# ParBLiSS/FastANI

Measured on AMD Instinct MI355X. Metric: ANI pairs/sec, many-to-many NxN ~5 Mbp genomes, higher is better.
Workload: dtype u32

## Files before the change

fastani_amd/csrc/engine_map.hip:

```cpp
#include <atomic>
#include <thread>
#include "host/engine.hpp"
#include "kernels/l1.hpp"
#include "kernels/l2.hpp"
#include "kernels/reduce.hpp"
#include "kernels/profile.hpp"
#include "kernels/cluster.hpp"
#include "kernels/tree.hpp"
#include "kernels/nj.hpp"
#include "kernels/single.hpp"
#include "kernels/sigdist.hpp"
#include "kernels/sigstrip.hpp"
#include "kernels/signeigh.hpp"
#include "kernels/sigscreen.hpp"
#include "kernels/sigcontain.hpp"
#include "kernels/sigcluster.hpp"
#include "kernels/siggraph.hpp"

namespace anih {
using namespace ani;

void launch_l2_codes(unsigned grid, hipStream_t s, const L2FastArgs &fa);
void launch_l2_sim_a(unsigned grid, hipStream_t s, const L2FastArgs &fa, const int32_t *list, const unsigned int *listCount);
void launch_l2_sim_b(unsigned grid, hipStream_t s, const L2FastArgs &fa, const int32_t *list, const unsigned int *listCount);
// ... 186 lines not shown
    TRY(device_scan(ctx, ctx->fragCandCntClamped.as<int32_t>(), ctx->fragOrdOff.as<uint32_t>(), (uint32_t)nF, &nCand));
    if (nCand) {
      TRY(ctx->ocFrag.ensure(nCand * 4)); TRY(ctx->ocSeq.ensure(nCand * 4)); TRY(ctx->ocStart.ensure(nCand * 4)); TRY(ctx->ocEnd.ensure(nCand * 4));
      hipLaunchKernelGGL(k_l1_order, dim3(grid_for(nF)), dim3(256), 0, ctx->stream, ctx->fragCandOff.as<uint32_t>(), ctx->fragCandCntClamped.as<int32_t>(),
                         ctx->fragOrdOff.as<uint32_t>(), fragOrder, (int32_t)nF, ctx->candSeq.as<int32_t>(), ctx->candStart.as<int32_t>(),
                             ctx->candEnd.as<int32_t>(),
                         ctx->ocFrag.as<int32_t>(), ctx->ocSeq.as<int32_t>(), ctx->ocStart.as<int32_t>(), ctx->ocEnd.as<int32_t>());
      HIP_TRY(hipGetLastError());
    }
  }
  *nCandOut = (int32_t)nCand;
  ctx->counters.l1Candidates += nCand;
  if (nCand == 0) return ANI_OK;

  TRY(ctx->l2Best.ensure(nCand * 4)); TRY(ctx->l2First.ensure(nCand * 4)); TRY(ctx->l2Last.ensure(nCand * 4));
  TRY(ctx->refStart.ensure(nCand * 4)); TRY(ctx->idBits.ensure(nCand * 4));
  {
    StageTimer tm(ctx, &ctx->counters.msL2);
    TRY(zero_counters(ctx));
    L2Args a;
    a.candFrag = ctx->ocFrag.as<int32_t>(); a.candSeq = ctx->ocSeq.as<int32_t>(); a.candStart = ctx->ocStart.as<int32_t>();
    a.candEnd = ctx->ocEnd.as<int32_t>();
    a.nCand = (int32_t)nCand; a.qPool = fs.qPool; a.fragOff = fs.fragOff; a.fragS = fs.fragS;
    a.mHash = sk->mHash; a.mWpos = sk->mWpos; a.dup = DupLinks{sk->dupList, sk->nDup, sk->dupBits}; a.mWin = sk->mWin; a.posBase = sk->posBase;
    a.posSample = sk->posSample;
    a.contigFirstMin = sk->contigFirstMin;
    { int lg = 0; while ((2 << lg) <= w) lg++; a.rankShift = 21 - std::max(0, lg - 1); }
    a.L = L; a.w = w; a.k = k; a.scratch = nullptr; a.laneStride = 0;
    a.outBest = ctx->l2Best.as<int32_t>(); a.outFirst = ctx->l2First.as<int32_t>(); a.outLast = ctx->l2Last.as<int32_t>();
    a.sumEntries = cnt_ptr(ctx, CNT_ENTRIES); a.sumSteps = cnt_ptr(ctx, CNT_STEPS); a.sumQ = cnt_ptr(ctx, CNT_SUMQ);

    uint32_t *ordOff = nullptr;
    TRY(pinned_buffer(ctx, 0, nF * 4, (void **)&ordOff));
    HIP_TRY(hipMemcpyAsync(ordOff, ctx->fragOrdOff.p, nF * 4, hipMemcpyDeviceToHost, ctx->stream));
    HIP_TRY(hipStreamSynchronize(ctx->stream));

    const size_t CH = ctx->l2ChunkCandidates;
    for (int p = 0; p < 2; p++) {
      TRY(ctx->l2Ranges[p].ensure(CH * sizeof(L2Range))); TRY(ctx->l2CodeCount[p].ensure(CH * 4)); TRY(ctx->l2CodeOff[p].ensure(CH * 4));
      TRY(ctx->l2SlowFlag[p].ensure(CH * 4)); TRY(ctx->l2ClassList[p].ensure(CH * 4));
      TRY(ctx->l2Order[p].ensure(CH * 4)); TRY(ctx->l2LenHist[p].ensure((kL2LenBuckets + 4) * 4));
    }
    TRY(ctx->l2SlowList.ensure(nCand * 4));
    HIP_TRY(hipMemsetAsync(cnt_ptr(ctx, CNT_NEG), 0, 8, ctx->stream));
    struct SideJoin { ani_ctx *c; ~SideJoin() { (void)hipStreamSynchronize(c->stream2); } } sideJoin{ctx};
    HIP_TRY(hipEventRecord(ctx->evSetDone[0], ctx->stream)); HIP_TRY(hipEventRecord(ctx->evSetDone[1], ctx->stream));
    HIP_TRY(hipStreamWaitEvent(ctx->stream2, ctx->evSetDone[1], 0));
    size_t chunk = CH;
    int nChunk = 0;
    for (size_t c0 = 0; c0 < nCand;) {
      const size_t c1 = std::min<size_t>(nCand, c0 + chunk);
      const size_t n = c1 - c0;
      const int p = nChunk & 1;
      HIP_TRY(hipEventSynchronize(ctx->evSetDone[p]));
      HIP_TRY(hipStreamWaitEvent(ctx->stream, ctx->evSetDone[p], 0));
      L2FastArgs fa;
      fa.g = a; fa.c0 = (int32_t)c0; fa.c1 = (int32_t)c1;
      fa.ranges = ctx->l2Ranges[p].as<L2Range>(); fa.codeCount = ctx->l2CodeCount[p].as<int32_t>(); fa.codeOff = ctx->l2CodeOff[p].as<uint32_t>();
      fa.codes = nullptr; fa.slowFlag = ctx->l2SlowFlag[p].as<int32_t>(); fa.fragCandOff = ctx->fragOrdOff.as<uint32_t>(); fa.fragOrder = fragOrder;
      fa.nFrag = (int32_t)nF;
      const int32_t fA = (int32_t)(std::upper_bound(ordOff, ordOff + nF, (uint32_t)c0) - ordOff) - 1;
      const int32_t fB = (int32_t)(std::upper_bound(ordOff, ordOff + nF, (uint32_t)(c1 - 1)) - ordOff) - 1;
      fa.fragBase = fA;
      { const char *ev = getenv("ANI_TEST_L2_PATH"); fa.allowFast = (ev && !strcmp(ev, "general")) ? 0 : (ev && !strcmp(ev, "classB")) ? 2 : 1; }
      if (L - (w - 1) - (k - 1) + 2 > (int)kWinMask || L - (w - 1) - (k - 1) < 1) fa.allowFast = 0;
      {
        StageTimer tk(ctx, &ctx->counters.msL2Ranges, 1);
        hipLaunchKernelGGL(k_l2_ranges, dim3(grid_for(n)), dim3(kTPB), 0, ctx->stream, fa);
      }
      fa.nFragChunk = fB - fA + 1;
      uint64_t nCodes = 0;
      {
        const int rc = device_scan(ctx, fa.codeCount, ctx->l2CodeOff[p].as<uint32_t>(), (uint32_t)n, &nCodes, ctx->l2CodeLimit);
        if (rc == ANI_ERR_LIMIT && n > 1) { chunk = (n + 1) / 2; ctx->counters.l2ChunkHalvings++; continue; }
        TRY(rc);
      }
      TRY(ctx->l2Codes[p].ensure((nCodes + 64) * 2));
      fa.codes = ctx->l2Codes[p].as<uint32_t>();
      if (nCodes) {
        {
          StageTimer tk(ctx, &ctx->counters.msL2Ranges, 1);
          HIP_TRY(hipMemsetAsync(ctx->l2LenHist[p].p, 0, kL2LenBuckets * 4, ctx->stream));
          HIP_TRY(hipMemsetD32Async((hipDeviceptr_t)(ctx->l2LenHist[p].as<unsigned int>() + kL2LenBuckets), (int)n, 1, ctx->stream));
          hipLaunchKernelGGL(k_l2_len_hist, dim3(grid_for(n, kTPB, 2048)), dim3(kTPB), 0, ctx->stream, (const int32_t *)fa.codeCount, (int32_t)n,
              ctx->l2LenHist[p].as<unsigned int>());
          hipLaunchKernelGGL(k_l2_len_scan, dim3(1), dim3(kTPB), 0, ctx->stream, ctx->l2LenHist[p].as<unsigned int>());
          hipLaunchKernelGGL(k_l2_len_scatter, dim3(grid_for(n, kTPB)), dim3(kTPB), 0, ctx->stream, (const int32_t *)fa.codeCount, (int32_t)c0, (int32_t)n,
                             ctx->l2LenHist[p].as<unsigned int>(), ctx->l2Order[p].as<int32_t>());
        }
        {
          StageTimer tk(ctx, &ctx->counters.msL2Codes, 1);
          launch_l2_codes((unsigned)((fa.nFragChunk + 7) / 8 * 8), ctx->stream, fa);
        }
        const bool overlap = ctx->l2Overlap;
        hipStream_t simStream = ctx->stream;
        if (overlap) {
          HIP_TRY(hipEventRecord(ctx->evSimA[p], ctx->stream));
          HIP_TRY(hipStreamWaitEvent(ctx->stream2, ctx->evSimA[p], 0));
          simStream = ctx->stream2;
        }
        {
          StageTimer tk(ctx, &ctx->counters.msL2Kernel, 1, simStream);
          launch_l2_sim_a(grid_for(n, kL2SimTPB), simStream, fa, (const int32_t *)ctx->l2Order[p].as<int32_t>(),
              (const unsigned int *)ctx->l2LenHist[p].as<unsigned int>() + kL2LenBuckets);
        }
        ctx->counters.l2Launches++;
      }
      HIP_TRY(hipEventRecord(ctx->evSimA[p], ctx->stream));
      HIP_TRY(hipStreamWaitEvent(ctx->stream2, ctx->evSimA[p], 0));
      if (nCodes) {
        StageTimer tk(ctx, &ctx->counters.msL2SimB, 1, ctx->stream2);
        HIP_TRY(hipMemsetAsync(cnt_ptr(ctx, CNT_CLASSB), 0, 8, ctx->stream2));
        hipLaunchKernelGGL(k_l2_collect_class, dim3(grid_for(n)), dim3(256), 0, ctx->stream2, (int32_t)c0, (int32_t)n, (const int32_t *)fa.slowFlag, 4,
                           ctx->l2ClassList[p].as<int32_t>(), (unsigned int *)cnt_ptr(ctx, CNT_CLASSB));
        L2FastArgs fb = fa;
        fb.g.sumEntries = cnt_ptr(ctx, CNT_ENTRIES_B); fb.g.sumQ = cnt_ptr(ctx, CNT_SUMQ_B); fb.g.sumSteps = cnt_ptr(ctx, CNT_STEPS_B);
        launch_l2_sim_b(grid_for(n, kL2SimTPB), ctx->stream2, fb, (const int32_t *)ctx->l2ClassList[p].as<int32_t>(), (const unsigned int *)cnt_ptr(ctx,
            CNT_CLASSB));
      }
      hipLaunchKernelGGL(k_l2_collect_slow, dim3(grid_for(n)), dim3(256), 0, ctx->stream2, (int32_t)c0, (int32_t)n, (const int32_t *)fa.slowFlag,
                         ctx->l2SlowList.as<int32_t>(), (unsigned int *)cnt_ptr(ctx, CNT_NEG), cnt_ptr(ctx, CNT_REASON));
      HIP_TRY(hipEventRecord(ctx->evSetDone[p], ctx->stream2));
      HIP_TRY(hipGetLastError());
      c0 = c1; nChunk++;
    }
    HIP_TRY(hipStreamWaitEvent(ctx->stream, ctx->evSetDone[0], 0)); HIP_TRY(hipStreamWaitEvent(ctx->stream, ctx->evSetDone[1], 0));
    unsigned long long nSlow64 = 0;
    HIP_TRY(hipMemcpyAsync(&nSlow64, cnt_ptr(ctx, CNT_NEG), 8, hipMemcpyDeviceToHost, ctx->stream));
    HIP_TRY(hipStreamSynchronize(ctx->stream));
    const size_t nSlowTotal = (size_t)(uint32_t)nSlow64;
    if (nSlowTotal) {
      size_t lanes = (std::min<size_t>(nSlowTotal, (size_t)1 << 17) + kTPB - 1) / kTPB * kTPB;
      const size_t wordsPerLane = (size_t)maxS + 1;
      while (lanes > kTPB && lanes * wordsPerLane * 4 > ((size_t)2 << 30)) lanes = (lanes / 2 + kTPB - 1) / kTPB * kTPB;
      TRY(ctx->l2Scratch.ensure(lanes * wordsPerLane * 4));
      L2Args sa = a; sa.scratch = ctx->l2Scratch.as<uint32_t>(); sa.laneStride = lanes;
      StageTimer tk(ctx, &ctx->counters.msL2Slow, 1);
      for (size_t base = 0; base < nSlowTotal; base += lanes)
        hipLaunchKernelGGL(k_l2, dim3((unsigned)(lanes / kTPB)), dim3(kTPB), 0, ctx->stream, sa, (const int32_t *)ctx->l2SlowList.as<int32_t>(),
            (int32_t)nSlowTotal, (int32_t)base);
      HIP_TRY(hipGetLastError());
    }
    ctx->counters.l2SlowCandidates += nSlowTotal; ctx->counters.l2FastCandidates += nCand - nSlowTotal;
    FinishArgs fa;
    fa.nCand = (int32_t)nCand; fa.candFrag = a.candFrag; fa.candSeq = a.candSeq; fa.best = a.outBest; fa.firstPos = a.outFirst; fa.lastPos = a.outLast;
    fa.fragS = a.fragS; fa.idLUT = set->dIdLUT; fa.minShared = set->dMinShared; fa.lutMaxS = set->dLutMaxS;
    fa.refStart = ctx->refStart.as<int32_t>(); fa.idBits = ctx->idBits.as<uint32_t>();
    hipLaunchKernelGGL(k_finish_candidates, dim3(grid_for(nCand)), dim3(256), 0, ctx->stream, fa);
    HIP_TRY(hipGetLastError());
  }
  TRY(read_counters(ctx, host));
  ctx->counters.l2WindowEntries += host[CNT_ENTRIES] + host[CNT_ENTRIES_B]; ctx->counters.l2Steps += host[CNT_STEPS] + host[CNT_STEPS_B];
  ctx->counters.l2QueryHashes += host[CNT_SUMQ] + host[CNT_SUMQ_B];
  ctx->counters.l2WindowEntriesB += host[CNT_ENTRIES_B]; ctx->counters.l2QueryHashesB += host[CNT_SUMQ_B];
  ctx->counters.l2SlowLimit += host[CNT_REASON + 1]; ctx->counters.l2SlowDup += host[CNT_REASON + 2]; ctx->counters.l2SlowOverflow += host[CNT_REASON + 3];
  return ANI_OK;
}

int reduce_stage(ani_ctx *ctx, ani_sketch *set, IndexChunk *sk, const FragSet &fs, int32_t nCand, int32_t nQuery, bool compact = false)
{
  if (nQuery == 0 || sk->nGenomes == 0) return ANI_OK;
  const size_t binsPerQuery = sk->totalBins;
  const size_t nBins = binsPerQuery * (size_t)nQuery;
  TRY(ctx->bins.ensure((nBins ? nBins : 1) * 4));
  const size_t nPairsAll = (size_t)nQuery * (size_t)(compact ? sk->nGenomes : set->nGenomes);
  TRY(ctx->rows.ensure((nPairsAll ? nPairsAll : 1) * 8));
  hipError_t e1;
  {
  StageTimer tm(ctx, &ctx->counters.msReduce);
  e1 = hipMemsetAsync(ctx->bins.p, 0, (nBins ? nBins : 1) * 4, ctx->stream);
// ... 1905 lines not shown
```

fastani_amd/csrc/kernels/l2.hpp:

```cpp
#pragma once
#include <type_traits>
#include "common.hpp"
#include "index.hpp"

namespace ani {

struct L2Result {
  int32_t best;
  int32_t firstPos;
  int32_t lastPos;
  int32_t entries;
  int32_t steps;
};

struct L2State {
  uint32_t *w;
  size_t stride;
  __host__ __device__ __forceinline__ uint32_t get(int g) const { return w[(size_t)g * stride]; }
  __host__ __device__ __forceinline__ void set(int g, uint32_t v) const { w[(size_t)g * stride] = v; }
};

__host__ __device__ __forceinline__ int32_t lower_bound_wpos(const int32_t *mWpos, int32_t lo, int32_t hi, int32_t pos)
{
  while (lo < hi) {
// ... 73 lines not shown
{
  L2Result r; r.best = 0; r.firstPos = 0; r.lastPos = 0; r.steps = 0;
  const int32_t cmw = L - (w - 1) - (k - 1);
  int32_t beg = lower_bound_wpos(mWpos, cLo, cHi, rangeStart);
  int32_t end = lower_bound_wpos(mWpos, cLo, cHi, mWpos[beg] + cmw);
  const int32_t last = lower_bound_wpos(mWpos, cLo, cHi, rangeEnd + L);
  r.entries = last - beg;
  L2Sim sim; sim.init(s, st);
  for (int32_t j = beg; j < end; j++)
    if (!dup_flag(dup, (uint32_t)j) || dup_prev(dup, (uint32_t)j) < beg) sim.insert(q_rank(q, s, mHash[j]));
  int32_t pb = beg, pe = end;
  int32_t pos = mWpos[beg];
  while (end < last) {
    if (pb != beg) {
      const int32_t nx = dup_flag(dup, (uint32_t)pb) ? dup_next(dup, (uint32_t)pb) : -1;
      if (!(nx >= 0 && nx < pe)) sim.erase(q_rank(q, s, mHash[pb]));
    }
    if (pe != end) {
      if (!dup_flag(dup, (uint32_t)pe) || dup_prev(dup, (uint32_t)pe) < beg) sim.insert(q_rank(q, s, mHash[pe]));
    }
    const int32_t wb = mWpos[beg];
    if (sim.shared > r.best) { r.best = sim.shared; r.firstPos = wb; r.lastPos = wb; }
    else if (sim.shared == r.best) r.lastPos = wb;
    r.steps++;
    pb = beg; pe = end;
    const int32_t d1 = mWpos[beg + 1] - pos;
    const int32_t d2 = mWpos[end] - (pos + cmw - 1);
    const int32_t adv = d1 < d2 ? d1 : d2;
    pos += adv;
    if (adv == d1) beg++;
    if (adv == d2) end++;
  }
  return r;
}

struct L2Args {
  const int32_t *candFrag, *candSeq, *candStart, *candEnd;
  int32_t nCand;
  const uint32_t *qPool; const uint32_t *fragOff; const int32_t *fragS;
  const uint32_t *mHash; const int32_t *mWpos; DupLinks dup;
  const uint32_t *mWin;
  const int32_t *contigFirstMin;
  const uint32_t *posBase, *posSample;
  int rankShift;
  int L, w, k;
  uint32_t *scratch; size_t laneStride;
  int32_t *outBest, *outFirst, *outLast;
  unsigned long long *sumEntries, *sumSteps, *sumQ;
};

static __global__ __launch_bounds__(kTPB) void k_l2(L2Args a, const int32_t *__restrict__ list, int32_t listCount, int32_t listBase)
{
  const int32_t lane = blockIdx.x * blockDim.x + threadIdx.x;
  const int32_t li = listBase + lane;
  unsigned long long e = 0, st = 0, sq = 0;
  if (li < listCount && (size_t)lane < a.laneStride) {
    const int32_t c = list ? list[li] : li;
    const int32_t f = a.candFrag[c];
    const int32_t seq = a.candSeq[c];
    L2State state; state.w = a.scratch + lane; state.stride = a.laneStride;
    L2Result r = l2_candidate(a.qPool + a.fragOff[f], a.fragS[f], a.mHash, a.mWpos, a.dup,
                              a.contigFirstMin[seq], a.contigFirstMin[seq + 1], a.candStart[c], a.candEnd[c],
                              a.L, a.w, a.k, state);
    a.outBest[c] = r.best; a.outFirst[c] = r.firstPos; a.outLast[c] = r.lastPos;
    e = (unsigned long long)r.entries; st = (unsigned long long)r.steps; sq = (unsigned long long)a.fragS[f];
  }
#pragma unroll
  for (int d = 32; d > 0; d >>= 1) { e += __shfl_down(e, d); st += __shfl_down(st, d); sq += __shfl_down(sq, d); }
  if ((threadIdx.x & 63) == 0 && (e | st | sq)) { atomicAdd(stat_slot(a.sumEntries), e); atomicAdd(stat_slot(a.sumSteps), st);
    atomicAdd(stat_slot(a.sumQ), sq); }
}

constexpr int kL2FastMaxS = 319;
constexpr int kL2FastMaxEntries = 16384;
template <int MAXS>
struct L2Geom {
  static constexpr int kMaxS = MAXS;
  static constexpr int kStateWords = (MAXS + 1 + 3) / 4;
  static constexpr int kWords = kStateWords;
};
using L2GeomA = L2Geom<255>;
using L2GeomB = L2Geom<319>;
constexpr int kL2SimTPB = 64;

struct L2Range { int32_t beg0, end0, last, nEvents; };

struct L2FastArgs {
  L2Args g;
  int32_t c0, c1;
  L2Range *ranges;
  int32_t *codeCount;
  const uint32_t *codeOff;
  uint32_t *codes;
  int32_t *slowFlag;
  const uint32_t *fragCandOff;
  const int32_t *fragOrder;
  int32_t nFrag, fragBase, nFragChunk;
  int32_t allowFast;
};

__device__ __forceinline__ int32_t l2_search_pos(const L2Args &g, uint32_t pb, int32_t nb, int32_t cHi, int32_t pos)
{
  int32_t bin = (pos < 0 ? 0 : pos) >> kPosSampleShift; bin = bin < nb ? bin : nb - 1;
  const int32_t lo = (int32_t)g.posSample[pb + (uint32_t)bin];
  const int32_t hi = bin + 1 < nb ? (int32_t)g.posSample[pb + (uint32_t)bin + 1] : cHi;
  return lower_bound_wpos(g.mWpos, lo, hi, pos);
}

static __global__ __launch_bounds__(kTPB) void k_l2_ranges(L2FastArgs a)
{
  const int32_t c = a.c0 + blockIdx.x * blockDim.x + threadIdx.x;
  if (c >= a.c1) return;
  const int32_t i = c - a.c0;
  const int32_t seq = a.g.candSeq[c];
  const int32_t cLo = a.g.contigFirstMin[seq], cHi = a.g.contigFirstMin[seq + 1];
  const int32_t cmw = a.g.L - (a.g.w - 1) - (a.g.k - 1);
  L2Range r;
  const uint32_t pb = a.g.posBase[seq]; const int32_t nb = (int32_t)(a.g.posBase[seq + 1] - pb);
  auto search = [&](int32_t pos) -> int32_t { return l2_search_pos(a.g, pb, nb, cHi, pos); };
  r.beg0 = search(a.g.candStart[c]);
  const int32_t wposBeg0 = a.g.mWpos[r.beg0];
  r.end0 = search(wposBeg0 + cmw);
  r.last = search(a.g.candEnd[c] + a.g.L);
  const int32_t m = r.last - r.beg0;
  const int32_t s = a.g.fragS[a.g.candFrag[c]];
  const bool fast = a.allowFast && s >= 1 && s <= kL2FastMaxS && m >= 1 && m <= kL2FastMaxEntries;
  int32_t nEv = 0;
  if (fast && r.end0 < r.last) {
    const int32_t lastDel = (r.last - 1) - (int32_t)(a.g.mWin[r.last - 1] & kWinMask) - 2;
    const int32_t nDel = lastDel >= r.beg0 ? lastDel - r.beg0 + 1 : 0;
    nEv = (r.end0 - r.beg0) + (r.last - 1 - r.end0) + nDel;
  }
  r.nEvents = nEv;
  a.ranges[i] = r;
  if (fast && nEv == 0) {
    a.g.outBest[c] = 0; a.g.outFirst[c] = 0; a.g.outLast[c] = 0;
    a.codeCount[i] = 0; a.slowFlag[i] = 16;
    return;
  }
  a.codeCount[i] = fast ? ((nEv + 8) & ~7) : 0;
  a.slowFlag[i] = fast ? ((s <= L2GeomA::kMaxS && a.allowFast != 2) ? 0 : 4) : 1;
}

constexpr uint32_t kL2DupBit = 1u << 10, kL2InsBit = 1u << 11, kL2NoEvalBit = 1u << 12;
constexpr int kL2DeltaShift = 13;
static_assert((kWinDupBit >> 21) == kL2DupBit && (kWinMoreBit >> 18) == kL2NoEvalBit, "flag bits of the window links shift into the event code");
constexpr int kL2RankBuckets = 2048;
__device__ __forceinline__ int l2_rank_bucket(uint32_t h, int sh) { const uint32_t b = h >> sh;
  return (int)(b < (uint32_t)(kL2RankBuckets - 1) ? b : (uint32_t)(kL2RankBuckets - 1)); }

__device__ __forceinline__ void l2_rank_table(const uint32_t *__restrict__ q, int s, int sh, uint32_t *qs, uint32_t *st2, uint32_t *cnt2, int *scanScratch)
{
  static_assert(kL2FastMaxS <= 2 * kTPB && kL2RankBuckets == 8 * kTPB, "two sketch hashes and eight buckets per thread");
  { uint4 z; z.x = z.y = z.z = z.w = 0u; ((uint4 *)cnt2)[threadIdx.x] = z; }
  const int i0 = (int)threadIdx.x, i1 = (int)threadIdx.x + kTPB;
  const uint32_t q0 = i0 < s ? q[i0] : 0xffffffffu, q1 = i1 < s ? q[i1] : 0xffffffffu;
  if (i0 < s) qs[i0] = q0;
  if (i1 < s) qs[i1] = q1;
  if (threadIdx.x < 2) qs[s + threadIdx.x] = 0xffffffffu;
  block_barrier();
  if (i0 < s) { const int b = l2_rank_bucket(q0, sh); atomicAdd(&cnt2[b >> 1], 1u << ((b & 1) << 4)); }
  if (i1 < s) { const int b = l2_rank_bucket(q1, sh); atomicAdd(&cnt2[b >> 1], 1u << ((b & 1) << 4)); }
  block_barrier();
  {
    const uint4 c4 = ((const uint4 *)cnt2)[threadIdx.x];
    const uint32_t cw[4] = {c4.x, c4.y, c4.z, c4.w};
    uint32_t n[8], loc[8], sum = 0;
#pragma unroll
    for (int j = 0; j < 8; j++) { n[j] = (j & 1) ? (cw[j >> 1] >> 16) : (cw[j >> 1] & 0xffffu); loc[j] = sum; sum += n[j]; }
    int tot;
    const uint32_t base = (uint32_t)block_excl_scan((int)sum, scanScratch, &tot);
    uint4 o0, o1;
    o0.x = (base + loc[0]) | (n[0] << 16); o0.y = (base + loc[1]) | (n[1] << 16); o0.z = (base + loc[2]) | (n[2] << 16); o0.w = (base + loc[3]) | (n[3] << 16);
    o1.x = (base + loc[4]) | (n[4] << 16); o1.y = (base + loc[5]) | (n[5] << 16); o1.z = (base + loc[6]) | (n[6] << 16); o1.w = (base + loc[7]) | (n[7] << 16);
    ((uint4 *)st2)[2 * threadIdx.x] = o0; ((uint4 *)st2)[2 * threadIdx.x + 1] = o1;
  }
  block_barrier();
}
__device__ __forceinline__ uint32_t l2_rank_fast(const uint32_t *qs, const uint32_t *st2, int sh, uint32_t h, uint32_t &deep)
{
  const uint32_t sp = st2[l2_rank_bucket(h, sh)];
  const uint32_t lo = sp & 0xffffu;
  const uint32_t q0 = qs[lo], q1 = qs[lo + 1];
  deep |= (uint32_t)(q1 < h) & (uint32_t)(sp > 0x2ffffu);
  return ((lo + (uint32_t)(q0 < h) + (uint32_t)(q1 < h)) << 1) | (uint32_t)((q0 == h) | (q1 == h));
}
__device__ __forceinline__ uint32_t l2_rank_deep(const uint32_t *qs, const uint32_t *st2, int sh, int s, uint32_t h, uint32_t rk)
{
  const uint32_t sp = st2[l2_rank_bucket(h, sh)];
  int lo = (int)(sp & 0xffffu), hi = lo + (int)(sp >> 16);
  if (hi - lo > 2) {
    while (lo < hi) { const int mid = (lo + hi) >> 1; if (qs[mid] < h) lo = mid + 1; else hi = mid; }
    rk = ((uint32_t)lo << 1) | (uint32_t)(lo < s && qs[lo] == h);
  }
  return rk;
}

constexpr int kL2StageEvents = 2048;
constexpr int kL2CandBatch = 40;
static __global__ __launch_bounds__(kTPB) void k_l2_codes(L2FastArgs a)
{
  __shared__ uint32_t qs[kL2FastMaxS + 2];
  __shared__ __attribute__((aligned(16))) uint32_t st2[kL2RankBuckets];
  __shared__ __attribute__((aligned(16))) uint16_t stageAll[(kTPB / kWave) * kL2StageEvents];
  __shared__ L2Range cRange[kL2CandBatch];
  __shared__ uint64_t cOff[kL2CandBatch];
  __shared__ int cRangeScan[8];
#ifdef ANI_L2C_PAD_WORDS
  __shared__ volatile uint32_t padLds[ANI_L2C_PAD_WORDS];
  if (threadIdx.x == 0) padLds[blockIdx.x & (ANI_L2C_PAD_WORDS - 1)] = 1u;
#endif
  const int32_t per = (int32_t)(gridDim.x >> 3);
  const int32_t fl = (int32_t)(blockIdx.x & 7) * per + (int32_t)(blockIdx.x >> 3);
  if (fl >= a.nFragChunk) return;
  const int32_t fi = a.fragBase + fl;
  const int32_t f = a.fragOrder ? a.fragOrder[fi] : fi;
  const int32_t s = a.g.fragS[f];
  int32_t cA = (int32_t)a.fragCandOff[fi], cB = (fi + 1 < a.nFrag) ? (int32_t)a.fragCandOff[fi + 1] : a.g.nCand;
  if (cA < a.c0) cA = a.c0;
  if (cB > a.c1) cB = a.c1;
  if (cA >= cB || s < 1 || s > kL2FastMaxS) return;
  const uint32_t *q = a.g.qPool + a.g.fragOff[f];
  auto fetch_cands = [&](int32_t base) {
    const int32_t c = base + (int32_t)threadIdx.x;
    if ((int)threadIdx.x < kL2CandBatch && c < cB) {
      const int32_t i = c - a.c0;
      L2Range r = a.ranges[i];
      if (a.codeCount[i] == 0) r.nEvents = -1;
      cRange[threadIdx.x] = r; cOff[threadIdx.x] = a.codeOff[i];
    }
  };
  fetch_cands(cA);
  const int sh = a.g.rankShift;
  l2_rank_table(q, s, sh, qs, st2, (uint32_t *)stageAll , cRangeScan);

  const int lane = threadIdx.x & (kWave - 1), wv = wave_uniform((int32_t)(threadIdx.x >> 6));
  uint16_t *stage = stageAll + wv * kL2StageEvents;
  struct Item {
    int32_t c; uint32_t jb;
    char *ob; const char *hb, *wb;
    uint32_t m, nInit, nInsAll, nDel, dump; bool staged, lastPass;
  };
  constexpr uint32_t kPass = 4u * kWave;
  int32_t batch0 = cA, batch1 = cA + kL2CandBatch < cB ? cA + kL2CandBatch : cB;
  auto open_cand = [&](int32_t c, Item &it) -> bool {
    for (; c < batch1; c += kTPB / kWave) {
      L2Range r = cRange[c - batch0];
      r.nEvents = wave_uniform(r.nEvents);
      if (r.nEvents < 0) continue;
      r.beg0 = wave_uniform(r.beg0); r.end0 = wave_uniform(r.end0); r.last = wave_uniform(r.last);
      it.c = c; it.jb = 0;
      it.ob = (char *)((uint16_t *)a.codes + wave_uniform(cOff[c - batch0]));
      it.hb = (const char *)(a.g.mHash + r.beg0); it.wb = (const char *)(a.g.mWin + r.beg0);
      it.m = (uint32_t)(r.last - r.beg0);
      it.nInit = (uint32_t)(r.end0 - r.beg0); it.nInsAll = it.m - 1;
      it.nDel = (uint32_t)r.nEvents - it.nInsAll;
      it.dump = (uint32_t)r.nEvents;
      it.staged = (uint32_t)r.nEvents < (uint32_t)kL2StageEvents;
      it.lastPass = kPass >= it.m;
      return true;
    }
    return false;
  };
  auto next_item = [&](const Item &cur, Item &nx) -> bool {
    if (!cur.lastPass) { nx = cur; nx.jb = cur.jb + kPass; nx.lastPass = nx.jb + kPass >= nx.m; return true; }
    return open_cand(cur.c + kTPB / kWave, nx);
  };
  auto load_item = [&](const Item &it, uint32_t (&h)[4], uint32_t (&wl)[4]) {
#pragma unroll
    for (int e = 0; e < 4; e++) {
      const uint32_t x = it.jb + lane + e * kWave;
      const uint32_t off = (x < it.m ? x : it.m - 1) * 4u;
      h[e] = *(const uint32_t *)(it.hb + off); wl[e] = *(const uint32_t *)(it.wb + off);
    }
  };
  Item cur, nxt;
  for (;;) {
  bool have = open_cand(batch0 + wv, cur);
  uint32_t h[4], wl[4], hn[4], wn[4];
  if (have) load_item(cur, h, wl);
  while (have) {
    const bool haveNext = next_item(cur, nxt);
    if (haveNext) load_item(nxt, hn, wn);
    auto pass_body = [&](auto eTag) {
      constexpr int E = decltype(eTag)::value;
      uint32_t rk[4];
      uint32_t deep = 0;
  #pragma unroll
      for (int e = 0; e < E; e++) rk[e] = l2_rank_fast(qs, st2, sh, h[e], deep);
      if (__any(deep != 0)) {
  #pragma unroll
        for (int e = 0; e < E; e++) rk[e] = l2_rank_deep(qs, st2, sh, s, h[e], rk[e]);
      }
      uint32_t pi[4], pd[4]; uint16_t ci[4], cdl[4];
      const uint32_t dumpSlot = cur.dump;
  #pragma unroll
      for (int e = 0; e < E; e++) {
        const uint32_t x = cur.jb + lane + e * kWave;
        const uint32_t cd = rk[e] | ((wl[e] >> 21) & kL2DupBit);
        const uint32_t mq = 0u - (rk[e] & 1u);
        const int32_t db = (int32_t)x - (int32_t)(wl[e] & kWinMask) - 1;
        pi[e] = x < cur.nInsAll ? x + (uint32_t)(db < 0 ? 0 : db) : dumpSlot;
        ci[e] = (uint16_t)((cd | kL2InsBit | (2u << kL2DeltaShift) | ((int32_t)x < (int32_t)cur.nInit - 1 ? kL2NoEvalBit : 0u)) ^ (mq & (3u << kL2DeltaShift)));
        const uint32_t ib = x + ((wl[e] >> kWinShiftA) & kWinMask);
        pd[e] = x < cur.nDel ? x + (ib < cur.nInit ? cur.nInit : ib) : dumpSlot;
        cdl[e] = (uint16_t)(cd | ((wl[e] >> 18) & kL2NoEvalBit) | (6u << kL2DeltaShift) | (mq & (1u << kL2DeltaShift)));
      }
      if (cur.staged) {
  #pragma unroll
        for (int e = 0; e < E; e++) { stage[pi[e]] = ci[e]; stage[pd[e]] = cdl[e]; }
      } else {
  #pragma unroll
        for (int e = 0; e < E; e++) { *(uint16_t *)(cur.ob + pi[e] * 2u) = ci[e]; *(uint16_t *)(cur.ob + pd[e] * 2u) = cdl[e]; }
      }
    };
    {
      const uint32_t left = cur.m - cur.jb;
      if (left > 3u * kWave) pass_body(std::integral_constant<int, 4>());
      else if (left > 2u * kWave) pass_body(std::integral_constant<int, 3>());
      else if (left > (uint32_t)kWave) pass_body(std::integral_constant<int, 2>());
      else pass_body(std::integral_constant<int, 1>());
    }
    if (cur.staged && cur.lastPass) {
      ANI_WAVE_SYNC();
      const uint32_t nOut = (cur.dump + 8u) & ~7u;
      for (uint32_t o = (uint32_t)lane * 8u; o < nOut; o += kWave * 8u) *(uint4 *)(cur.ob + o * 2u) = *(const uint4 *)(stage + o);
      ANI_WAVE_SYNC();
    }
    have = haveNext;
    if (have) {
      cur = nxt;
#pragma unroll
      for (int e = 0; e < 4; e++) { h[e] = hn[e]; wl[e] = wn[e]; }
    }
  }
  if (batch1 >= cB) break;
  block_barrier();
  fetch_cands(batch1);
  batch0 = batch1; batch1 = batch0 + kL2CandBatch < cB ? batch0 + kL2CandBatch : cB;
  block_barrier();
  }
}

struct L2Regs { int s, iStar, tot, shared; uint32_t ovfAcc; };
constexpr bool kL2ByteInterleave = true;
__device__ __forceinline__ int l2_field_off(int g) { return kL2ByteInterleave ? (g << 6) : (((g >> 2) << 8) + (g & 3)); }

__device__ __forceinline__ void l2_apply(uint8_t *F, L2Regs &r, uint32_t code, bool INS, bool on)
{
  const bool isQ = (code & 1u) != 0;
  const int idx = (int)((code >> 1) & 0x1ffu);
  const int d0 = ((int)(code << (32 - kL2DeltaShift - 3))) >> 29;
  const int d = on ? d0 : 0;
  const int sg = INS ? 1 : -1;
  int j = r.iStar - (INS ? 1 : 0); j = j < 0 ? 0 : j;
  uint8_t *pOwn = F + l2_field_off(idx);
  const int own = *pOwn;
  int fj = F[l2_field_off(j)];
  const int nw = own + d;
  r.ovfAcc |= (uint32_t)nw;
  *pOwn = (uint8_t)nw;
  fj += (idx == j) ? d : 0;
  const int c1 = (fj >> 1) + 1;
  const bool lt = idx < r.iStar;
  const int t = (on && lt) ? sg : 0;
  r.shared += isQ ? t : 0;
  r.tot += isQ ? 0 : t;
  const int reach = INS ? r.tot : r.tot + c1;
  const bool over = reach > r.s;
  const bool room = (INS ? idx : r.iStar) < (INS ? r.iStar : r.s);
  const bool mv = on && !isQ && room && (over == INS);
  const int mvm = -(int)mv;
  const int mone = sg & mvm;
  r.iStar -= mone;
  r.shared -= mone & -(fj & 1);
  r.tot -= (INS ? c1 : -c1) & mvm;
}

typedef uint32_t L2Block __attribute__((vector_size(16)));
__device__ __forceinline__ L2Block l2_block_zero() { const L2Block b = {0u, 0u, 0u, 0u}; return b; }
__device__ __forceinline__ L2Block l2_block_load(bool on, const uint4 *p, L2Block otherwise)
{
  if (on) otherwise = *(const L2Block *)p;
  return otherwise;
}
template <class G>
static __global__ __launch_bounds__(kL2SimTPB) void k_l2_sim(L2FastArgs a, const int32_t *__restrict__ list, const unsigned int *__restrict__ listCount)
{
  __shared__ uint32_t lds[(kL2SimTPB / kWave) * G::kWords * kWave];
  const int lane = threadIdx.x & (kWave - 1), wv = threadIdx.x >> 6;
  uint32_t *W = lds + wv * (G::kWords * kWave);
  uint8_t *F = (uint8_t *)W + (kL2ByteInterleave ? lane : 4 * lane);
  uint32_t *S = W + lane;
  const int32_t slot = blockIdx.x * blockDim.x + threadIdx.x;
  int32_t c = a.c0 + slot;
  if (list) {
    const unsigned int n = *listCount;
    if ((unsigned int)(blockIdx.x * blockDim.x) >= n) return;
    c = (unsigned int)slot < n ? list[slot] : a.c1;
  }
#pragma unroll
  for (int x = 0; x < G::kStateWords; x++) S[x * kWave] = 0u;
  unsigned long long cntE = 0, cntS = 0, cntQ = 0;
  const int myFlag = c < a.c1 ? a.slowFlag[c - a.c0] : 1;
  const bool mine = (G::kMaxS == 255) ? (myFlag == 0) : (myFlag == 4);
  const int32_t i = mine ? c - a.c0 : 0;
  L2Range r; r.beg0 = 0; r.end0 = 0; r.last = 0; r.nEvents = 0;
  if (mine) r = a.ranges[i];
  const int n = r.nEvents;
  L2Regs R; R.s = mine ? a.g.fragS[a.g.candFrag[c]] : 1; R.iStar = R.s; R.tot = R.s; R.shared = 0; R.ovfAcc = 0;
  const uint4 *p = (const uint4 *)((const uint16_t *)a.codes + (mine ? a.codeOff[i] : 0u));
  const int nBlk = (n + 7) >> 3;
  int best = 0, begAtBest = -1, begAtLast = -1, steps = 0, delCount = 0;
  L2Block cur = l2_block_load(mine, p, l2_block_zero());
  auto run_block = [&](auto plainTag, int blk, const L2Block &blkWords) {
    constexpr bool PLAIN = decltype(plainTag)::value;
    const uint32_t wd[4] = {blkWords[0], blkWords[1], blkWords[2], blkWords[3]};
#pragma unroll
    for (int e = 0; e < 8; e++) {
      const uint32_t code = (e & 1) ? (wd[e >> 1] >> 16) : (wd[e >> 1] & 0xffffu);
      const int ev = 8 * blk + e;
      const bool on = PLAIN ? true : ev < n;
      const bool INS = (code & kL2InsBit) != 0;
      bool eff = on;
      if (!PLAIN) {
        if (__any(on && (code & kL2DupBit) != 0)) {
          if (on && (code & kL2DupBit)) {
            const int insCount = ev - delCount;
            if (INS) eff = dup_prev(a.g.dup, (uint32_t)(r.beg0 + insCount)) < r.beg0 + delCount;
            else { const int32_t nx = dup_next(a.g.dup, (uint32_t)(r.beg0 + delCount)); eff = !(nx >= 0 && nx < r.beg0 + insCount); }
          }
        }
      }
      l2_apply(F, R, code, INS, eff);
      delCount += (on && !INS) ? 1 : 0;
      const bool evl = on && (code & kL2NoEvalBit) == 0;
      const int se = evl ? R.shared : -1;
      const bool better = se > best, tieOrBetter = se >= best;
      best = better ? R.shared : best;
      begAtBest = better ? delCount : begAtBest;
      begAtLast = tieOrBetter ? delCount : begAtLast;
      steps += evl ? 1 : 0;
    }
  };
  int blk = 0;
  {
    constexpr uint32_t kFillPair = (kL2InsBit | kL2NoEvalBit) * 0x10001u, kDupPair = kL2DupBit * 0x10001u;
    for (; __any(mine); blk++) {
      const uint32_t andw = cur[0] & cur[1] & cur[2] & cur[3], orw = cur[0] | cur[1] | cur[2] | cur[3];
      const bool fill = 8 * blk + 8 <= n && (andw & kFillPair) == kFillPair;
      if (!__all(fill || !mine)) break;
      const int nb = blk + 1 < nBlk ? blk + 1 : blk;
      const L2Block nxt = l2_block_load(mine, p + nb, cur);
      const bool anyDup = __any(mine && (orw & kDupPair) != 0);
      if (mine) {
        const uint32_t wd[4] = {cur[0], cur[1], cur[2], cur[3]};
#pragma unroll
        for (int e = 0; e < 8; e++) {
          const uint32_t code = (e & 1) ? (wd[e >> 1] >> 16) : (wd[e >> 1] & 0xffffu);
          int d = (int)((code >> kL2DeltaShift) & 7u);
          if (anyDup && (code & kL2DupBit) && dup_prev(a.g.dup, (uint32_t)(r.beg0 + 8 * blk + e)) >= r.beg0) d = 0;
          uint8_t *pOwn = F + l2_field_off((int)((code >> 1) & 0x1ffu));
          const int nw = (int)*pOwn + d;
          R.ovfAcc |= (uint32_t)nw;
          *pOwn = (uint8_t)nw;
        }
      }
      cur = nxt;
    }
    if (blk > 0) {
      int iS = 0, tot = 0, sh = 0, acc = 0; bool open = mine;
      for (int i = 1; __any(open && i <= R.s); i++) {
        const int f = F[l2_field_off(i - 1)];
        acc += f >> 1;
        open = open && i <= R.s && i + acc <= R.s;
        iS = open ? i : iS; tot = open ? i + acc : tot; sh += open ? (f & 1) : 0;
      }
      R.iStar = mine ? iS : R.iStar; R.tot = mine ? tot : R.tot; R.shared = mine ? sh : R.shared;
    }
  }
  for (; __any(blk < nBlk); blk++) {
    const int nb = blk + 1 < nBlk ? blk + 1 : blk;
    const L2Block nxt = l2_block_load(mine, p + nb, cur);
    const uint32_t orw = cur[0] | cur[1] | cur[2] | cur[3];
    const bool plain = !mine || (8 * blk + 8 <= n && (orw & (kL2DupBit | (kL2DupBit << 16))) == 0);
    if (__all(plain)) run_block(std::true_type(), blk, cur);
    else run_block(std::false_type(), blk, cur);
    cur = nxt;
  }
  if (mine) {
    if (R.ovfAcc & 0x100u) a.slowFlag[i] = 3;
    else {
      a.slowFlag[i] = (G::kMaxS == 255) ? 0 : 8;
      a.g.outBest[c] = best;
      a.g.outFirst[c] = begAtBest >= 0 ? a.g.mWpos[r.beg0 + begAtBest] : 0;
      a.g.outLast[c] = begAtLast >= 0 ? a.g.mWpos[r.beg0 + begAtLast] : 0;
      cntE = (unsigned long long)(r.last - r.beg0); cntS = (unsigned long long)steps; cntQ = (unsigned long long)R.s;
    }
  }
#pragma unroll
  for (int d = 32; d > 0; d >>= 1) { cntE += __shfl_down(cntE, d); cntS += __shfl_down(cntS, d); cntQ += __shfl_down(cntQ, d); }
  if (lane == 0 && (cntE | cntS | cntQ)) { atomicAdd(stat_slot(a.g.sumEntries), cntE); atomicAdd(stat_slot(a.g.sumSteps), cntS);
    atomicAdd(stat_slot(a.g.sumQ), cntQ); }
}



static __global__ void k_l2_collect_slow(int32_t c0, int32_t n, const int32_t *__restrict__ slowFlag, int32_t *__restrict__ list,
                                  unsigned int *__restrict__ count, unsigned long long *__restrict__ reasons )
{
  const int i = blockIdx.x * blockDim.x + threadIdx.x;
  if (i < n && (slowFlag[i] & 3)) { list[atomicAdd(count, 1u)] = c0 + i; atomicAdd(&reasons[slowFlag[i] & 3], 1ull); }
}

constexpr int kL2LenBuckets = 1024;
static __global__ __launch_bounds__(kTPB) void k_l2_len_hist(const int32_t *__restrict__ codeCount, int32_t n, unsigned int *__restrict__ hist)
{
  __shared__ unsigned int h[kL2LenBuckets];
  for (int i = threadIdx.x; i < kL2LenBuckets; i += kTPB) h[i] = 0;
  block_barrier();
  for (int i = blockIdx.x * kTPB + threadIdx.x; i < n; i += gridDim.x * kTPB) {
    int b = codeCount[i] >> 5; b = b >= kL2LenBuckets ? kL2LenBuckets - 1 : b;
    atomicAdd(&h[kL2LenBuckets - 1 - b], 1u);
  }
  block_barrier();
  for (int i = threadIdx.x; i < kL2LenBuckets; i += kTPB) if (h[i]) atomicAdd(&hist[i], h[i]);
}
static __global__ __launch_bounds__(kTPB) void k_l2_len_scan(unsigned int *__restrict__ hist)
{
  __shared__ int ws[16];
  block_array_excl_scan((int *)hist, kL2LenBuckets, ws);
}
static __global__ __launch_bounds__(kTPB) void k_l2_len_scatter(const int32_t *__restrict__ codeCount, int32_t c0, int32_t n,
                                                         unsigned int *__restrict__ cursor, int32_t *__restrict__ order)
{
  __shared__ unsigned int cnt[kL2LenBuckets], base[kL2LenBuckets];
  for (int i = threadIdx.x; i < kL2LenBuckets; i += kTPB) cnt[i] = 0;
  block_barrier();
  const int i = blockIdx.x * kTPB + threadIdx.x;
  int b = 0; unsigned int r = 0;
  if (i < n) {
    b = codeCount[i] >> 5; b = b >= kL2LenBuckets ? kL2LenBuckets - 1 : b;
    b = kL2LenBuckets - 1 - b;
    r = atomicAdd(&cnt[b], 1u);
  }
  block_barrier();
  for (int j = threadIdx.x; j < kL2LenBuckets; j += kTPB) if (cnt[j]) base[j] = atomicAdd(&cursor[j], cnt[j]);
  block_barrier();
  if (i < n) order[base[b] + r] = c0 + i;
}

static __global__ void k_l2_collect_class(int32_t c0, int32_t n, const int32_t *__restrict__ slowFlag, int32_t flag, int32_t *__restrict__ list,
                                   unsigned int *__restrict__ count)
{
  const int i = blockIdx.x * blockDim.x + threadIdx.x;
  if (i < n && slowFlag[i] == flag) list[atomicAdd(count, 1u)] = c0 + i;
}

}
```

Baseline: 5.230 million.

## Precompute initial window histogram in code generator instead of replaying fill events

The code-generation kernel now builds the initial window's per-sketch-slot histogram in shared memory with atomics and writes it as a packed state header before the event stream. The simulation kernel loads this state directly and computes the initial iStar/tot/shared prefix with byte sums, instead of replaying the fill events one by one. This shrinks the event stream and removes the serial fill phase from the simulation kernel. In exchange the generator does extra shared-memory atomics and dup checks, the stage buffer per wave gets smaller, and there is an overflow fallback to the slow path.

```diff
diff --git a/fastani_amd/csrc/engine_map.hip b/fastani_amd/csrc/engine_map.hip
--- a/fastani_amd/csrc/engine_map.hip
+++ b/fastani_amd/csrc/engine_map.hip
@@ -292,10 +292,10 @@
           StageTimer tk(ctx, &ctx->counters.msL2Ranges, 1);
           HIP_TRY(hipMemsetAsync(ctx->l2LenHist[p].p, 0, kL2LenBuckets * 4, ctx->stream));
           HIP_TRY(hipMemsetD32Async((hipDeviceptr_t)(ctx->l2LenHist[p].as<unsigned int>() + kL2LenBuckets), (int)n, 1, ctx->stream));
-          hipLaunchKernelGGL(k_l2_len_hist, dim3(grid_for(n, kTPB, 2048)), dim3(kTPB), 0, ctx->stream, (const int32_t *)fa.codeCount, (int32_t)n,
+          hipLaunchKernelGGL(k_l2_len_hist, dim3(grid_for(n, kTPB, 2048)), dim3(kTPB), 0, ctx->stream, (const L2Range *)fa.ranges, (int32_t)n,
               ctx->l2LenHist[p].as<unsigned int>());
           hipLaunchKernelGGL(k_l2_len_scan, dim3(1), dim3(kTPB), 0, ctx->stream, ctx->l2LenHist[p].as<unsigned int>());
-          hipLaunchKernelGGL(k_l2_len_scatter, dim3(grid_for(n, kTPB)), dim3(kTPB), 0, ctx->stream, (const int32_t *)fa.codeCount, (int32_t)c0, (int32_t)n,
+          hipLaunchKernelGGL(k_l2_len_scatter, dim3(grid_for(n, kTPB)), dim3(kTPB), 0, ctx->stream, (const L2Range *)fa.ranges, (int32_t)c0, (int32_t)n,
                              ctx->l2LenHist[p].as<unsigned int>(), ctx->l2Order[p].as<int32_t>());
         }
         {
diff --git a/fastani_amd/csrc/kernels/l2.hpp b/fastani_amd/csrc/kernels/l2.hpp
--- a/fastani_amd/csrc/kernels/l2.hpp
+++ b/fastani_amd/csrc/kernels/l2.hpp
@@ -179,6 +179,7 @@
 using L2GeomA = L2Geom<255>;
 using L2GeomB = L2Geom<319>;
 constexpr int kL2SimTPB = 64;
+__host__ __device__ __forceinline__ int l2_state_entries(bool classA) { return 2 * (classA ? L2GeomA::kStateWords : L2GeomB::kStateWords); }
 
 struct L2Range { int32_t beg0, end0, last, nEvents; };
 
@@ -226,7 +227,7 @@
   if (fast && r.end0 < r.last) {
     const int32_t lastDel = (r.last - 1) - (int32_t)(a.g.mWin[r.last - 1] & kWinMask) - 2;
     const int32_t nDel = lastDel >= r.beg0 ? lastDel - r.beg0 + 1 : 0;
-    nEv = (r.end0 - r.beg0) + (r.last - 1 - r.end0) + nDel;
+    nEv = 1 + (r.last - 1 - r.end0) + nDel;
   }
   r.nEvents = nEv;
   a.ranges[i] = r;
@@ -235,8 +236,9 @@
     a.codeCount[i] = 0; a.slowFlag[i] = 16;
     return;
   }
-  a.codeCount[i] = fast ? ((nEv + 8) & ~7) : 0;
-  a.slowFlag[i] = fast ? ((s <= L2GeomA::kMaxS && a.allowFast != 2) ? 0 : 4) : 1;
+  const bool classA = s <= L2GeomA::kMaxS && a.allowFast != 2;
+  a.codeCount[i] = fast ? l2_state_entries(classA) + ((nEv + 8) & ~7) : 0;
+  a.slowFlag[i] = fast ? (classA ? 0 : 4) : 1;
 }
 
 constexpr uint32_t kL2DupBit = 1u << 10, kL2InsBit = 1u << 11, kL2NoEvalBit = 1u << 12;
@@ -293,13 +295,16 @@
   return rk;
 }
 
-constexpr int kL2StageEvents = 2048;
+constexpr int kL2WaveWindow = 2048;
+constexpr int kL2HistWords = (kL2FastMaxS + 1) / 2;
+constexpr int kL2StageEvents = kL2WaveWindow - 2 * kL2HistWords;
+static_assert(kL2HistWords == 2 * L2GeomB::kStateWords && (kL2HistWords & 3) == 0 && L2GeomB::kStateWords <= 2 * kWave, "histogram: two dwords per state dword, 16-byte multiple, two state dwords per lane");
 constexpr int kL2CandBatch = 40;
 static __global__ __launch_bounds__(kTPB) void k_l2_codes(L2FastArgs a)
 {
   __shared__ uint32_t qs[kL2FastMaxS + 2];
   __shared__ __attribute__((aligned(16))) uint32_t st2[kL2RankBuckets];
-  __shared__ __attribute__((aligned(16))) uint16_t stageAll[(kTPB / kWave) * kL2StageEvents];
+  __shared__ __attribute__((aligned(16))) uint16_t stageAll[(kTPB / kWave) * kL2WaveWindow];
   __shared__ L2Range cRange[kL2CandBatch];
   __shared__ uint64_t cOff[kL2CandBatch];
   __shared__ int cRangeScan[8];
@@ -332,11 +337,17 @@
   l2_rank_table(q, s, sh, qs, st2, (uint32_t *)stageAll , cRangeScan);
 
   const int lane = threadIdx.x & (kWave - 1), wv = wave_uniform((int32_t)(threadIdx.x >> 6));
-  uint16_t *stage = stageAll + wv * kL2StageEvents;
+  uint32_t *hist = (uint32_t *)(stageAll + wv * kL2WaveWindow);
+  uint16_t *stage = stageAll + wv * kL2WaveWindow + 2 * kL2HistWords;
+  const bool classA = s <= L2GeomA::kMaxS && a.allowFast != 2;
+  const int stateWords = classA ? L2GeomA::kStateWords : L2GeomB::kStateWords;
+  for (int x = lane; x < stateWords; x += kWave) { hist[2 * x] = 0u; hist[2 * x + 1] = 0u; }
+  ANI_WAVE_SYNC();
   struct Item {
     int32_t c; uint32_t jb;
     char *ob; const char *hb, *wb;
     uint32_t m, nInit, nInsAll, nDel, dump; bool staged, lastPass;
+    uint32_t K; int32_t beg0;
   };
   constexpr uint32_t kPass = 4u * kWave;
   int32_t batch0 = cA, batch1 = cA + kL2CandBatch < cB ? cA + kL2CandBatch : cB;
@@ -347,11 +358,12 @@
       if (r.nEvents < 0) continue;
       r.beg0 = wave_uniform(r.beg0); r.end0 = wave_uniform(r.end0); r.last = wave_uniform(r.last);
       it.c = c; it.jb = 0;
-      it.ob = (char *)((uint16_t *)a.codes + wave_uniform(cOff[c - batch0]));
+      it.ob = (char *)((uint16_t *)a.codes + wave_uniform(cOff[c - batch0]) + (uint64_t)(2 * stateWords));
       it.hb = (const char *)(a.g.mHash + r.beg0); it.wb = (const char *)(a.g.mWin + r.beg0);
       it.m = (uint32_t)(r.last - r.beg0);
       it.nInit = (uint32_t)(r.end0 - r.beg0); it.nInsAll = it.m - 1;
-      it.nDel = (uint32_t)r.nEvents - it.nInsAll;
+      it.K = it.nInit - 1u; it.beg0 = r.beg0;
+      it.nDel = (uint32_t)r.nEvents + it.K - it.nInsAll;
       it.dump = (uint32_t)r.nEvents;
       it.staged = (uint32_t)r.nEvents < (uint32_t)kL2StageEvents;
       it.lastPass = kPass >= it.m;
@@ -389,6 +401,25 @@
   #pragma unroll
         for (int e = 0; e < E; e++) rk[e] = l2_rank_deep(qs, st2, sh, s, h[e], rk[e]);
       }
+      if (cur.jb < cur.K) {
+        uint32_t dl[4] = {0u, 0u, 0u, 0u}; uint32_t dupAny = 0;
+  #pragma unroll
+        for (int e = 0; e < E; e++) {
+          const uint32_t x0 = cur.jb + e * kWave;
+          if (x0 >= cur.K) continue;
+          const uint32_t d = 2u - (rk[e] & 1u);
+          if (x0 + kWave <= cur.K) { dl[e] = d; dupAny |= wl[e]; }
+          else { const bool in = x0 + lane < cur.K; dl[e] = in ? d : 0u; dupAny |= in ? wl[e] : 0u; }
+        }
+        if (__any((dupAny & kWinDupBit) != 0)) {
+  #pragma unroll
+          for (int e = 0; e < E; e++)
+            if (dl[e] && (wl[e] & kWinDupBit) && dup_prev(a.g.dup, (uint32_t)cur.beg0 + cur.jb + lane + e * kWave) >= cur.beg0) dl[e] = 0u;
+        }
+  #pragma unroll
+        for (int e = 0; e < E; e++)
+          if (cur.jb + e * kWave < cur.K) atomicAdd(&hist[rk[e] >> 2], dl[e] << ((rk[e] & 2u) << 3));
+      }
       uint32_t pi[4], pd[4]; uint16_t ci[4], cdl[4];
       const uint32_t dumpSlot = cur.dump;
   #pragma unroll
@@ -396,19 +427,22 @@
         const uint32_t x = cur.jb + lane + e * kWave;
         const uint32_t cd = rk[e] | ((wl[e] >> 21) & kL2DupBit);
         const uint32_t mq = 0u - (rk[e] & 1u);
-        const int32_t db = (int32_t)x - (int32_t)(wl[e] & kWinMask) - 1;
-        pi[e] = x < cur.nInsAll ? x + (uint32_t)(db < 0 ? 0 : db) : dumpSlot;
-        ci[e] = (uint16_t)((cd | kL2InsBit | (2u << kL2DeltaShift) | ((int32_t)x < (int32_t)cur.nInit - 1 ? kL2NoEvalBit : 0u)) ^ (mq & (3u << kL2DeltaShift)));
+        pi[e] = dumpSlot; ci[e] = 0;
+        if (cur.jb + (uint32_t)(e + 1) * kWave > cur.K) {
+          const int32_t db = (int32_t)x - (int32_t)(wl[e] & kWinMask) - 1;
+          pi[e] = x - cur.K < cur.nInsAll - cur.K ? x - cur.K + (uint32_t)(db < 0 ? 0 : db) : dumpSlot;
+          ci[e] = (uint16_t)((cd | kL2InsBit | (2u << kL2DeltaShift)) ^ (mq & (3u << kL2DeltaShift)));
+        }
         const uint32_t ib = x + ((wl[e] >> kWinShiftA) & kWinMask);
-        pd[e] = x < cur.nDel ? x + (ib < cur.nInit ? cur.nInit : ib) : dumpSlot;
+        pd[e] = x < cur.nDel ? x + (ib < cur.nInit ? cur.nInit : ib) - cur.K : dumpSlot;
         cdl[e] = (uint16_t)(cd | ((wl[e] >> 18) & kL2NoEvalBit) | (6u << kL2DeltaShift) | (mq & (1u << kL2DeltaShift)));
       }
       if (cur.staged) {
   #pragma unroll
-        for (int e = 0; e < E; e++) { stage[pi[e]] = ci[e]; stage[pd[e]] = cdl[e]; }
+        for (int e = 0; e < E; e++) { if (cur.jb + (uint32_t)(e + 1) * kWave > cur.K) stage[pi[e]] = ci[e]; stage[pd[e]] = cdl[e]; }
       } else {
   #pragma unroll
-        for (int e = 0; e < E; e++) { *(uint16_t *)(cur.ob + pi[e] * 2u) = ci[e]; *(uint16_t *)(cur.ob + pd[e] * 2u) = cdl[e]; }
+        for (int e = 0; e < E; e++) { if (cur.jb + (uint32_t)(e + 1) * kWave > cur.K) *(uint16_t *)(cur.ob + pi[e] * 2u) = ci[e]; *(uint16_t *)(cur.ob + pd[e] * 2u) = cdl[e]; }
       }
     };
     {
@@ -418,6 +452,19 @@
       else if (left > (uint32_t)kWave) pass_body(std::integral_constant<int, 2>());
       else pass_body(std::integral_constant<int, 1>());
     }
+    if (cur.jb + kPass >= cur.K && (cur.jb == 0u || cur.jb < cur.K)) {
+      ANI_WAVE_SYNC();
+      uint32_t *state = (uint32_t *)cur.ob - stateWords;
+      uint32_t ovf = 0;
+      for (int x = lane; x < stateWords; x += kWave) {
+        const uint32_t c0 = hist[2 * x], c1 = hist[2 * x + 1];
+        hist[2 * x] = 0u; hist[2 * x + 1] = 0u;
+        ovf |= (c0 | c1) & 0xff00ff00u;
+        state[x] = perm_b32(c1, c0, 0x06040200u);
+      }
+      if (__any(ovf != 0) && lane == 0) a.slowFlag[cur.c - a.c0] = 3;
+      ANI_WAVE_SYNC();
+    }
     if (cur.staged && cur.lastPass) {
       ANI_WAVE_SYNC();
       const uint32_t nOut = (cur.dump + 8u) & ~7u;
@@ -440,7 +487,11 @@
 }
 
 struct L2Regs { int s, iStar, tot, shared; uint32_t ovfAcc; };
+#ifdef ANI_L2_WORD_INTERLEAVE
+constexpr bool kL2ByteInterleave = false;
+#else
 constexpr bool kL2ByteInterleave = true;
+#endif
 __device__ __forceinline__ int l2_field_off(int g) { return kL2ByteInterleave ? (g << 6) : (((g >> 2) << 8) + (g & 3)); }
 
 __device__ __forceinline__ void l2_apply(uint8_t *F, L2Regs &r, uint32_t code, bool INS, bool on)
@@ -475,6 +526,14 @@
 }
 
 typedef uint32_t L2Block __attribute__((vector_size(16)));
+__device__ __forceinline__ uint32_t l2_byte_sum(uint32_t x, uint32_t acc)
+{
+#if defined(__HIP_DEVICE_COMPILE__)
+  return __builtin_amdgcn_sad_u8(x, 0u, acc);
+#else
+  return acc + (x & 0xffu) + ((x >> 8) & 0xffu) + ((x >> 16) & 0xffu) + (x >> 24);
+#endif
+}
 __device__ __forceinline__ L2Block l2_block_zero() { const L2Block b = {0u, 0u, 0u, 0u}; return b; }
 __device__ __forceinline__ L2Block l2_block_load(bool on, const uint4 *p, L2Block otherwise)
 {
@@ -496,8 +555,6 @@
     if ((unsigned int)(blockIdx.x * blockDim.x) >= n) return;
     c = (unsigned int)slot < n ? list[slot] : a.c1;
   }
-#pragma unroll
-  for (int x = 0; x < G::kStateWords; x++) S[x * kWave] = 0u;
   unsigned long long cntE = 0, cntS = 0, cntQ = 0;
   const int myFlag = c < a.c1 ? a.slowFlag[c - a.c0] : 1;
   const bool mine = (G::kMaxS == 255) ? (myFlag == 0) : (myFlag == 4);
@@ -505,8 +562,41 @@
   L2Range r; r.beg0 = 0; r.end0 = 0; r.last = 0; r.nEvents = 0;
   if (mine) r = a.ranges[i];
   const int n = r.nEvents;
-  L2Regs R; R.s = mine ? a.g.fragS[a.g.candFrag[c]] : 1; R.iStar = R.s; R.tot = R.s; R.shared = 0; R.ovfAcc = 0;
+  const int nHand = mine ? r.end0 - r.beg0 - 1 : 0;
   const uint4 *p = (const uint4 *)((const uint16_t *)a.codes + (mine ? a.codeOff[i] : 0u));
+  L2Regs R; R.s = mine ? a.g.fragS[a.g.candFrag[c]] : 1; R.ovfAcc = 0;
+  int accN = 0, accFull = 0, nFull = 0, shFull = 0;
+#pragma unroll
+  for (int x4 = 0; x4 < G::kStateWords / 4; x4++) {
+    L2Block v = l2_block_zero();
+    if (mine) v = *(const L2Block *)(p + x4);
+#pragma unroll
+    for (int y = 0; y < 4; y++) {
+      const uint32_t dw = v[y];
+      const int x = 4 * x4 + y;
+      if (kL2ByteInterleave) {
+#pragma unroll
+        for (int b = 0; b < 4; b++) F[l2_field_off(4 * x + b)] = (uint8_t)(dw >> (8 * b));
+      } else S[x * kWave] = dw;
+      accN = (int)l2_byte_sum((dw >> 1) & 0x7f7f7f7fu, (uint32_t)accN);
+      const bool full = 4 * (x + 1) + accN <= R.s;
+      nFull += full ? 1 : 0;
+      accFull = full ? accN : accFull;
+      shFull += full ? __popc(dw & 0x01010101u) : 0;
+    }
+  }
+  p += G::kStateWords / 4;
+  {
+    int run = accFull, below = accFull, cnt = 0, sh = shFull;
+#pragma unroll
+    for (int j = 0; j < 4; j++) {
+      const int f = F[l2_field_off(4 * nFull + j)];
+      run += f >> 1;
+      const bool ok = 4 * nFull + j + 1 + run <= R.s;
+      below = ok ? run : below; cnt += ok ? 1 : 0; sh += ok ? (f & 1) : 0;
+    }
+    R.iStar = 4 * nFull + cnt; R.tot = R.iStar + below; R.shared = sh;
+  }
   const int nBlk = (n + 7) >> 3;
   int best = 0, begAtBest = -1, begAtLast = -1, steps = 0, delCount = 0;
   L2Block cur = l2_block_load(mine, p, l2_block_zero());
@@ -523,7 +613,7 @@
       if (!PLAIN) {
         if (__any(on && (code & kL2DupBit) != 0)) {
           if (on && (code & kL2DupBit)) {
-            const int insCount = ev - delCount;
+            const int insCount = nHand + ev - delCount;
             if (INS) eff = dup_prev(a.g.dup, (uint32_t)(r.beg0 + insCount)) < r.beg0 + delCount;
             else { const int32_t nx = dup_next(a.g.dup, (uint32_t)(r.beg0 + delCount)); eff = !(nx >= 0 && nx < r.beg0 + insCount); }
           }
@@ -541,41 +631,6 @@
     }
   };
   int blk = 0;
-  {
-    constexpr uint32_t kFillPair = (kL2InsBit | kL2NoEvalBit) * 0x10001u, kDupPair = kL2DupBit * 0x10001u;
-    for (; __any(mine); blk++) {
-      const uint32_t andw = cur[0] & cur[1] & cur[2] & cur[3], orw = cur[0] | cur[1] | cur[2] | cur[3];
-      const bool fill = 8 * blk + 8 <= n && (andw & kFillPair) == kFillPair;
-      if (!__all(fill || !mine)) break;
-      const int nb = blk + 1 < nBlk ? blk + 1 : blk;
-      const L2Block nxt = l2_block_load(mine, p + nb, cur);
-      const bool anyDup = __any(mine && (orw & kDupPair) != 0);
-      if (mine) {
-        const uint32_t wd[4] = {cur[0], cur[1], cur[2], cur[3]};
-#pragma unroll
-        for (int e = 0; e < 8; e++) {
-          const uint32_t code = (e & 1) ? (wd[e >> 1] >> 16) : (wd[e >> 1] & 0xffffu);
-          int d = (int)((code >> kL2DeltaShift) & 7u);
-          if (anyDup && (code & kL2DupBit) && dup_prev(a.g.dup, (uint32_t)(r.beg0 + 8 * blk + e)) >= r.beg0) d = 0;
-          uint8_t *pOwn = F + l2_field_off((int)((code >> 1) & 0x1ffu));
-          const int nw = (int)*pOwn + d;
-          R.ovfAcc |= (uint32_t)nw;
-          *pOwn = (uint8_t)nw;
-        }
-      }
-      cur = nxt;
-    }
-    if (blk > 0) {
-      int iS = 0, tot = 0, sh = 0, acc = 0; bool open = mine;
-      for (int i = 1; __any(open && i <= R.s); i++) {
-        const int f = F[l2_field_off(i - 1)];
-        acc += f >> 1;
-        open = open && i <= R.s && i + acc <= R.s;
-        iS = open ? i : iS; tot = open ? i + acc : tot; sh += open ? (f & 1) : 0;
-      }
-      R.iStar = mine ? iS : R.iStar; R.tot = mine ? tot : R.tot; R.shared = mine ? sh : R.shared;
-    }
-  }
   for (; __any(blk < nBlk); blk++) {
     const int nb = blk + 1 < nBlk ? blk + 1 : blk;
     const L2Block nxt = l2_block_load(mine, p + nb, cur);
@@ -611,14 +666,14 @@
 }
 
 constexpr int kL2LenBuckets = 1024;
-static __global__ __launch_bounds__(kTPB) void k_l2_len_hist(const int32_t *__restrict__ codeCount, int32_t n, unsigned int *__restrict__ hist)
+__device__ __forceinline__ int l2_len_bucket(const L2Range &r) { const int b = ((r.nEvents + 8) & ~7) >> 5; return b >= kL2LenBuckets ? kL2LenBuckets - 1 : b; }
+static __global__ __launch_bounds__(kTPB) void k_l2_len_hist(const L2Range *__restrict__ ranges, int32_t n, unsigned int *__restrict__ hist)
 {
   __shared__ unsigned int h[kL2LenBuckets];
   for (int i = threadIdx.x; i < kL2LenBuckets; i += kTPB) h[i] = 0;
   block_barrier();
   for (int i = blockIdx.x * kTPB + threadIdx.x; i < n; i += gridDim.x * kTPB) {
-    int b = codeCount[i] >> 5; b = b >= kL2LenBuckets ? kL2LenBuckets - 1 : b;
-    atomicAdd(&h[kL2LenBuckets - 1 - b], 1u);
+    atomicAdd(&h[kL2LenBuckets - 1 - l2_len_bucket(ranges[i])], 1u);
   }
   block_barrier();
   for (int i = threadIdx.x; i < kL2LenBuckets; i += kTPB) if (h[i]) atomicAdd(&hist[i], h[i]);
@@ -628,7 +683,7 @@
   __shared__ int ws[16];
   block_array_excl_scan((int *)hist, kL2LenBuckets, ws);
 }
-static __global__ __launch_bounds__(kTPB) void k_l2_len_scatter(const int32_t *__restrict__ codeCount, int32_t c0, int32_t n,
+static __global__ __launch_bounds__(kTPB) void k_l2_len_scatter(const L2Range *__restrict__ ranges, int32_t c0, int32_t n,
                                                          unsigned int *__restrict__ cursor, int32_t *__restrict__ order)
 {
   __shared__ unsigned int cnt[kL2LenBuckets], base[kL2LenBuckets];
@@ -637,8 +692,7 @@
   const int i = blockIdx.x * kTPB + threadIdx.x;
   int b = 0; unsigned int r = 0;
   if (i < n) {
-    b = codeCount[i] >> 5; b = b >= kL2LenBuckets ? kL2LenBuckets - 1 : b;
-    b = kL2LenBuckets - 1 - b;
+    b = kL2LenBuckets - 1 - l2_len_bucket(ranges[i]);
     r = atomicAdd(&cnt[b], 1u);
   }
   block_barrier();
```

Result: faster. 5.309 million (median of 6 runs) (+1.5%).
